# qq456cvb/CanonicalVoting

Hardware: AMD Instinct MI355X
Metric: scenes/sec (80k-pt synthetic scans) (higher is better)
Workload: dtype f32

## Files before the change

### canonicalvoting_amd/csrc/hv_vote.hip

```cpp
#include "cv_common.h"

#include <atomic>
#include <algorithm>
#include <cmath>
#include <cstddef>
#include <mutex>
#include <unordered_map>
#include <vector>

namespace {

struct F3 { float x, y, z; };
struct I3 { int x, y, z; };

std::mutex g_tab_mu;
std::unordered_map<uint64_t, float2*> g_tabs;

int get_rot_table(int num_rots, const float2** out) {
    int dev = 0;
    CV_HIP_CHECK(hipGetDevice(&dev));
    const uint64_t key = (uint64_t(uint32_t(dev)) << 32) | uint32_t(num_rots);
    std::lock_guard<std::mutex> lk(g_tab_mu);
    auto it = g_tabs.find(key);
    if (it != g_tabs.end()) { *out = it->second; return CV_OK; }
// ... 207 lines not shown
constexpr int MAX_PARTS = HV_MAX_PARTS;

template <class V, class E>
__device__ __forceinline__ int wave_excl_scan(int Y, V value, E emit) {
    const int lane = threadIdx.x & 63;
    int carry = 0;
    for (int base = 0; base < Y; base += 64) {
        const int i = base + lane;
        const int v = i < Y ? value(i) : 0;
        int incl = v;
#pragma unroll
        for (int off = 1; off < 64; off <<= 1) {
            const int t = __shfl_up(incl, off);
            if (lane >= off) incl += t;
        }
        if (i < Y) emit(i, carry + incl - v, v);
        carry += __shfl(incl, 63);
    }
    return carry;
}
__global__ __launch_bounds__(256) void hv_prep_scan(const int* __restrict__ ycount, int Y,
                                                    int* __restrict__ ystart,
                                                    int* __restrict__ cursor,
                                                    int* __restrict__ part_start, int4* __restrict__ q_info, int max_q,
                                                    int* __restrict__ chunk_start, int* __restrict__ bin_of_chunk,
                                                    int part_records, int64_t ks_ws) {
    ycount = cat_ws(ycount, ks_ws); ystart = cat_ws(ystart, ks_ws); cursor = cat_ws(cursor, ks_ws);
    part_start = cat_ws(part_start, ks_ws); q_info = cat_ws(q_info, ks_ws);
    chunk_start = cat_ws(chunk_start, ks_ws); bin_of_chunk = cat_ws(bin_of_chunk, ks_ws);
    const int wave = threadIdx.x >> 6, lane = threadIdx.x & 63;
    if (wave == 0) {
        const int total = wave_excl_scan(Y, [&](int i) { return ycount[i]; },
                                         [&](int i, int excl, int) { ystart[i] = excl; cursor[i] = excl; });
        if (lane == 0) ystart[Y] = total;
    } else if (wave == 1) {
        const int total = wave_excl_scan(Y,
            [&](int i) {
                const int n2 = (i >= 1 ? ycount[i - 1] : 0) + (i <= Y - 2 ? ycount[i] : 0);
                return min(max((n2 + part_records - 1) / part_records, 1), MAX_PARTS);
            },
            [&](int i, int excl, int v) {
                part_start[i] = excl;
                for (int p2 = 0; p2 < v; ++p2) q_info[excl + p2] = make_int4(i, p2, v, excl);
            });
        for (int q = total + lane; q < max_q; q += 64) q_info[q] = make_int4(0, 0, -1, 0);
        if (lane == 0) part_start[Y] = total;
    } else if (wave == 2) {
        const int total = wave_excl_scan(Y, [&](int i) { return (ycount[i] + LIST_CHUNK_RECORDS - 1) / LIST_CHUNK_RECORDS; },
                                         [&](int i, int excl, int v) {
                                             chunk_start[i] = excl;
                                             for (int p2 = 0; p2 < v; ++p2) bin_of_chunk[excl + p2] = i;
                                         });
        if (lane == 0) chunk_start[Y] = total;
    }
}

constexpr int REC_F = 13;

__global__ __launch_bounds__(PREP_THREADS) void hv_prep_scatter(
    const float* __restrict__ pts, const float* __restrict__ xyz, const float* __restrict__ scl,
    const float* __restrict__ obj, const int* __restrict__ fy_in, int64_t n, int Y, float res,
    F3 corner, int* __restrict__ cursor, float* __restrict__ rec, int64_t rec_stride, CatStride ks) {
    __shared__ int lh[PREP_MAX_Y];
    xyz = cat_el(xyz, 3 * ks.n); scl = cat_el(scl, 3 * ks.n); obj = cat_el(obj, ks.n);
    fy_in = cat_ws(fy_in, ks.ws); cursor = cat_ws(cursor, ks.ws); rec = cat_ws(rec, ks.ws);
    const bool use_lds = Y <= PREP_MAX_Y;
    const int64_t c = blockIdx.x * (int64_t)PREP_THREADS + threadIdx.x;
// ... 380 lines not shown
        if (ok && hi - lo > best) { best = hi - lo; best_end = (float)k * half_pi + hi; }
#pragma unroll
        for (int j = 1; j < 4; ++j) {
            const float hp = h[(k + j - 1) & 3], hn = h[(k + j) & 3];
            ok = ok && hn > 0.f && hp + hn >= half_pi;
            if (ok) {
                lo = fminf(lo, (float)j * half_pi - hn);
                hi = fmaxf(hi, (float)j * half_pi + hn);
                if (hi - lo > best) { best = hi - lo; best_end = (float)k * half_pi + hi; }
            }
        }
    }
    const float inside = fmaxf(two_pi - best, 0.f);
    const float inv_step = (float)R * 0.159154943f;
    const int len = (int)(inside * inv_step) + 6;
    if (len < a_len) {
        float first = (best_end - a0) * inv_step - 2.f;
        first -= (float)R * floorf(first / (float)R);
        a_start = min(max((int)first, 0), R - 1);
        a_len = len;
    }
}

template <int VARIANT, bool QUEUE>
__global__ __launch_bounds__(TW * 64) void hv_fwd_tiles(
    int R, float res, F3 corner, I3 dims, const float2* __restrict__ tab,
    const int* __restrict__ ystart, const int4* __restrict__ items, const float* __restrict__ rec,
    int64_t rec_stride, int tiles_x, int tiles_z, unsigned long long* __restrict__ partials,
    int* __restrict__ arrivals, float* __restrict__ g_obj, float* __restrict__ g_rot,
    float* __restrict__ g_scale, unsigned long long* __restrict__ prof,
    const int* __restrict__ list_ctl, const int* __restrict__ list_start, const int* __restrict__ list_cnt,
    const int2* __restrict__ entries, int list_mode ,
    const int4* __restrict__ q_info, CatStride ks) {
    ystart = cat_ws(ystart, ks.ws); items = cat_ws(items, ks.ws); rec = cat_ws(rec, ks.ws);
    partials = cat_ws(partials, ks.ws); arrivals = cat_ws(arrivals, ks.ws); list_ctl = cat_ws(list_ctl, ks.ws);
    list_start = cat_ws(list_start, ks.ws); list_cnt = cat_ws(list_cnt, ks.ws); entries = cat_ws(entries, ks.ws);
    q_info = cat_ws(q_info, ks.ws);
    g_obj = cat_el(g_obj, ks.cells); g_rot = cat_el(g_rot, 2 * ks.cells); g_scale = cat_el(g_scale, 3 * ks.cells);
    __shared__ TileShared sh;
    __shared__ int last_flag;
    unsigned long long pacc[8] = {0, 0, 0, 0, 0, 0, 0, 0};
    unsigned long long pt0 = VARIANT == 4 ? __builtin_amdgcn_s_memtime() : 0;
#define HV_TICK(p)                                                        \
    do {                                                                  \
        if (VARIANT == 4) {                                               \
            const unsigned long long t_ = __builtin_amdgcn_s_memtime();   \
            pacc[p] += t_ - pt0;                                          \
            pt0 = t_;                                                     \
        }                                                                 \
    } while (0)
    const int X = dims.x, Y = dims.y, Z = dims.z;
    const int ntiles = tiles_x * tiles_z;
    int y, tile, part, nparts, slot0, slot_stride;
    if (QUEUE) {
        if ((int)blockIdx.x >= list_ctl[2]) return;
        const int4 item = items[blockIdx.x];
        y = item.x; tile = item.y; part = item.z & 0xff; nparts = item.z >> 8; slot0 = item.w; slot_stride = 1;
    } else {
        tile = blockIdx.x % ntiles;
        const int4 qi = q_info[blockIdx.x / ntiles];
        if (qi.z < 0) return;
        y = qi.x; part = qi.y; nparts = qi.z;
        slot0 = qi.w * ntiles + tile; slot_stride = ntiles;
    }
    const int x0 = (tile / tiles_z) * TX, z0 = (tile % tiles_z) * TZ;
    const int lane = threadIdx.x & 63, wave = threadIdx.x >> 6;
    if (nparts == 0) {
        const int nx0 = min(TX, X - x0), nz0 = min(TZ, Z - z0);
        for (int i = threadIdx.x; i < TCELLS; i += TW * 64) {
            const int lx = i / TZ, lz = i % TZ;
            if (lx < nx0 && lz < nz0) {
                const int64_t cell = ((int64_t)(x0 + lx) * Y + y) * Z + z0 + lz;
                g_obj[cell] = 0.f;
                reinterpret_cast<float2*>(g_rot)[cell] = make_float2(0.f, 0.f);
                g_scale[cell * 3 + 0] = 0.f; g_scale[cell * 3 + 1] = 0.f; g_scale[cell * 3 + 2] = 0.f;
            }
        }
        return;
    }
    const bool use_list = QUEUE && VARIANT != 3 && list_mode == 2 && list_ctl[1] == 0;
    int lbeg[2] = {0, 0}, llen[2] = {0, 0};
    if (use_list) {
#pragma unroll
        for (int k = 0; k < 2; ++k) {
            const int s = y - 1 + k;
            if (s >= 0 && s <= Y - 2) {
                lbeg[k] = list_start[(int64_t)s * ntiles + tile];
                llen[k] = list_cnt[(int64_t)s * ntiles + tile];
            }
        }
    }

#ifdef HV_POISON
    {
        unsigned* w = reinterpret_cast<unsigned*>(&sh);
        const int lo[5] = {(int)(offsetof(TileShared, pq) / 4), (int)(offsetof(TileShared, arc_start) / 4),
                           (int)(offsetof(TileShared, arc_cum) / 4), (int)(offsetof(TileShared, vq_rec) / 4),
                           (int)(offsetof(TileShared, tab) / 4)};
        const int hi[5] = {lo[1], lo[2], lo[3], lo[4], (int)(offsetof(TileShared, next_chunk) / 4)};
        for (int k = 0; k < 5; ++k)
            if ((HV_POISON >> k) & 1)
                for (int i = lo[k] + threadIdx.x; i < hi[k]; i += TW * 64) w[i] = 0x7fc12345u + i * 2654435761u;
        __syncthreads();
    }
#endif
    int bin_beg[2], bin_end[2];
#pragma unroll
    for (int k = 0; k < 2; ++k) {
        const int s = y - 1 + k;
        const bool valid = s >= 0 && s <= Y - 2 && VARIANT != 3;
        bin_beg[k] = !valid ? 0 : (use_list ? lbeg[k] : ystart[s]);
        bin_end[k] = !valid ? 0 : (use_list ? lbeg[k] + llen[k] : ystart[s + 1]);
    }
    const float2 tab_mine = (int)threadIdx.x < R ? tab[threadIdx.x] : make_float2(0.f, 0.f);
    for (int i = threadIdx.x; i < ACC_WORDS; i += TW * 64) sh.acc[i] = 0ull;
    if ((int)threadIdx.x < R) sh.tab[threadIdx.x] = tab_mine;
    if (threadIdx.x < 2) sh.next_chunk[threadIdx.x] = 0;
    if (threadIdx.x == 2) { sh.list_len = 0; sh.more = 0; }
    __syncthreads();
    HV_TICK(0);

    const float slack = 0.05f;
    const float xlo = (float)(x0 - 1), xhi = (float)(x0 + TX), zlo = (float)(z0 - 1),
                zhi = (float)(z0 + TZ);
    int vq_len = 0;

    const int per = use_list ? LIST_CHUNK : 64;
    int sb = 0;
    int c_mask = 0, c_idx[CULL_BATCH], c_arc = 0, c_k = 0;
#pragma unroll
    for (int j = 0; j < CULL_BATCH; ++j) c_idx[j] = 0;
    auto append = [&](int mask, const int (&idx)[CULL_BATCH], int arc, int k) -> int {
        int tot = 0, before[CULL_BATCH];
#pragma unroll
        for (int j = 0; j < CULL_BATCH; ++j) {
            const uint64_t m = __ballot((mask >> j) & 1);
            before[j] = tot + lanes_below(m);
            tot += __popcll(m);
        }
        if (tot == 0) return 0;
        int p0 = 0;
        if (lane == 0) p0 = atomicAdd(&sh.list_len, tot);
        p0 = __builtin_amdgcn_readfirstlane(p0);
#pragma unroll
        for (int j = 0; j < CULL_BATCH; ++j) {
            const int pos = p0 + before[j];
            if (((mask >> j) & 1) && pos < LQ) {
                sh.arc_start[pos] = idx[j] | (int)((unsigned)k << 31);
                if (use_list) sh.arc_cum[pos] = arc;
                mask &= ~(1 << j);
            }
        }
        return mask;
    };

    for (;;) {
        bool more = false;
        if (__ballot(c_mask != 0) != 0) {
            c_mask = append(c_mask, c_idx, c_arc, c_k);
            more = __ballot(c_mask != 0) != 0;
        }
        while (!more && sb < 2) {
            if (bin_beg[sb] >= bin_end[sb]) { ++sb; continue; }
            const int len = __builtin_amdgcn_readfirstlane(
                __hip_atomic_load(&sh.list_len, __ATOMIC_RELAXED, __HIP_MEMORY_SCOPE_WORKGROUP));
            if (len > LQ - 64) { more = true; break; }
            const int take = use_list ? 64 / LIST_CHUNK : CULL_BATCH;
            int c = 0;
            if (lane == 0) c = atomicAdd(&sh.next_chunk[sb], take);
            c = __builtin_amdgcn_readfirstlane(c);
            const int end = bin_end[sb];
            if (bin_beg[sb] + (c * nparts + part) * per >= end) { ++sb; continue; }
            int idx[CULL_BATCH], mask = 0, arc = 0;
#pragma unroll
            for (int j = 0; j < CULL_BATCH; ++j) idx[j] = 0;
            if (use_list) {
                const int e = bin_beg[sb] + ((c + lane / LIST_CHUNK) * nparts + part) * LIST_CHUNK + lane % LIST_CHUNK;
                if (e < end) {
// ... 19 lines not shown
                    const float dxf = fmaxf(fabsf(ux[j] - xlo), fabsf(ux[j] - xhi));
                    const float dzf = fmaxf(fabsf(uz[j] - zlo), fabsf(uz[j] - zhi));
                    const float dmin = sqrtf(dxn * dxn + dzn * dzn), dmax = sqrtf(dxf * dxf + dzf * dzf);
                    const float tol = slack + 1e-5f * (r[j] + fabsf(ux[j]) + fabsf(uz[j]));
                    bool keep = idx[j] < end && (r[j] >= dmin - tol) && (r[j] <= dmax + tol);
                    if (VARIANT == 2) keep = keep && (ux[j] == 1234.5f);
                    mask |= (int)keep << j;
                }
            }
            c_mask = append(mask, idx, arc, sb);
            if (__ballot(c_mask != 0) != 0) {
#pragma unroll
                for (int j = 0; j < CULL_BATCH; ++j) c_idx[j] = idx[j];
                c_arc = arc; c_k = sb;
                more = true;
            }
        }
        if (more && lane == 0) sh.more = 1;
        HV_TICK(1);
        __syncthreads();
        const int n = min(sh.list_len, LQ);
        const bool again = sh.more != 0;
        HV_TICK(3);
        if (n == 0) break;

        const int p = threadIdx.x;
        int a_start = 0, a_len = 0;
        if (p < n) {
            const int w = sh.arc_start[p];
            const int idx = w & 0x7fffffff;
            if (use_list) {
                const int arc = sh.arc_cum[p];
                a_start = arc & 0xffff;
                a_len = arc >> 16;
            } else {
                const float ux = rec[9 * rec_stride + idx], uz = rec[10 * rec_stride + idx];
                const float dxn = fmaxf(0.f, fmaxf(xlo - ux, ux - xhi));
                const float dzn = fmaxf(0.f, fmaxf(zlo - uz, uz - zhi));
                a_len = R;
                if (dxn + dzn > 0.5f) {
                    const float b0 = arc_atan2(0.5f * (zlo + zhi) - uz, 0.5f * (xlo + xhi) - ux);
                    float lo = 0.f, hi = 0.f;
#pragma unroll
                    for (int k = 0; k < 4; ++k) {
                        float d = arc_atan2(((k & 2) ? zhi : zlo) - uz, ((k & 1) ? xhi : xlo) - ux) - b0;
                        d -= 6.28318531f * rintf(d * 0.159154943f);
                        lo = fminf(lo, d);
                        hi = fmaxf(hi, d);
                    }
                    const float a0 = rec[12 * rec_stride + idx];
                    const float inv_step = (float)R * 0.159154943f;
                    float first = (b0 + lo - a0) * inv_step - 2.f;
                    const int len = (int)((hi - lo) * inv_step) + 6;
                    first -= (float)R * floorf(first / (float)R);
                    a_start = min(max((int)first, 0), R - 1);
                    a_len = min(len, R);
                }
                edge_arc(ux, uz, rec[11 * rec_stride + idx], rec[12 * rec_stride + idx], R, xlo, xhi, zlo, zhi, a_start, a_len);
            }
            const float ry = rec[4 * rec_stride + idx];
            sh.pq[0][p] = rec[0 * rec_stride + idx];
            sh.pq[1][p] = rec[1 * rec_stride + idx];
            sh.pq[2][p] = rec[2 * rec_stride + idx];
            sh.pq[3][p] = rec[3 * rec_stride + idx];
            sh.pq[4][p] = (w < 0) ? (1.f - ry) : ry;
            sh.pq[5][p] = rec[5 * rec_stride + idx];
            sh.pq[6][p] = rec[6 * rec_stride + idx];
            sh.pq[7][p] = rec[7 * rec_stride + idx];
            sh.pq[8][p] = rec[8 * rec_stride + idx];
            sh.arc_start[p] = a_start;
        }
        int cum = a_len;
#pragma unroll
        for (int off = 1; off < 64; off <<= 1) {
            const int t = __shfl_up(cum, off);
            if (lane >= off) cum += t;
        }
        if (lane == 63) sh.wtot[wave] = cum;
        HV_TICK(2);
        __syncthreads();
        HV_TICK(3);
        if (threadIdx.x == 0) { sh.list_len = 0; sh.more = 0; }
        int items = 0;
#pragma unroll
        for (int w = 0; w < TW; ++w) {
            const int t = sh.wtot[w];
            if (w < wave) cum += t;
            items += t;
        }
        if (p < n) sh.arc_cum[p] = cum;
        HV_TICK(2);
        __syncthreads();
// ... 64 lines not shown
                sh.vq_rz[wave][q] = rz;
            }
            vq_len += __popcll(mv);
            wave_sync_lds();
            HV_TICK(4);
            if (vq_len >= 64) {
                vq_len -= 64;
                if (VARIANT != 1) drain64(sh, wave, vq_len + lane, true);
                HV_TICK(5);
            }
        }
        if (vq_len > 0) {
            if (VARIANT != 1) drain64(sh, wave, lane, lane < vq_len);
            else if (lane < vq_len)
                sh.acc[ACC_CH + lane] = (unsigned long long)(sh.vq_rx[wave][lane] + sh.vq_rz[wave][lane] + (float)sh.vq_rec[wave][lane]);
            vq_len = 0;
        }
        wave_sync_lds();
        HV_TICK(6);
        if (!again) break;
        __syncthreads();
        HV_TICK(3);
    }
    HV_TICK(1);
    __syncthreads();
    HV_TICK(3);

    if (nparts > 1) {
        unsigned long long* mine = partials + ((int64_t)slot0 + (int64_t)part * slot_stride) * (6 * TCELLS);
        for (int i = threadIdx.x; i < 6 * TCELLS; i += TW * 64) mine[i] = sh.acc[acc_idx(i / TCELLS, i % TCELLS)];
        asm volatile("s_waitcnt vmcnt(0)" ::: "memory");
        __syncthreads();
        if (threadIdx.x == 0) {
            __builtin_amdgcn_fence(__ATOMIC_RELEASE, "agent");
            asm volatile("s_waitcnt vmcnt(0)" ::: "memory");
            const int old = __hip_atomic_fetch_add(&arrivals[y * ntiles + tile], 1, __ATOMIC_RELAXED,
                                                   __HIP_MEMORY_SCOPE_AGENT);
            last_flag = old == nparts - 1;
            if (last_flag) __builtin_amdgcn_fence(__ATOMIC_ACQUIRE, "agent");
        }
        __syncthreads();
        if (!last_flag) return;
        const unsigned long long* base = partials + (int64_t)slot0 * (6 * TCELLS);
        for (int i = threadIdx.x; i < 6 * TCELLS; i += TW * 64) {
            unsigned long long sum = 0ull;
            for (int p2 = 0; p2 < nparts; ++p2) sum += base[(int64_t)p2 * slot_stride * (6 * TCELLS) + i];
            sh.acc[acc_idx(i / TCELLS, i % TCELLS)] = sum;
        }
        __syncthreads();
    }

    const int nx = min(TX, X - x0), nz = min(TZ, Z - z0);
    if (VARIANT == 5) {
        if (threadIdx.x == 0) g_obj[((int64_t)x0 * Y + y) * Z + z0] = (float)acc_value(sh.acc[0], 0);
        return;
    }
    for (int i = threadIdx.x; i < TCELLS; i += TW * 64) {
        const int lx = i / TZ, lz = i % TZ;
        if (lx < nx && lz < nz)
            g_obj[((int64_t)(x0 + lx) * Y + y) * Z + z0 + lz] = (float)acc_value(sh.acc[acc_idx(0, i)], 0);
    }
    for (int i = threadIdx.x; i < TCELLS * 2; i += TW * 64) {
        const int cell = i >> 1, j = i & 1;
        const int lx = cell / TZ, lz = cell % TZ;
        if (lx < nx && lz < nz) {
            const double d = (double)(float)acc_value(sh.acc[acc_idx(0, cell)], 0) + 1e-7;
            g_rot[(((int64_t)(x0 + lx) * Y + y) * Z + z0 + lz) * 2 + j] =
                (float)((double)(float)fx_value(sh.acc[acc_idx(1 + j, cell)]) / d);
        }
    }
    for (int i = threadIdx.x; i < TCELLS * 3; i += TW * 64) {
        const int cell = i / 3, j = i - cell * 3;
        const int lx = cell / TZ, lz = cell % TZ;
        if (lx < nx && lz < nz) {
            const double d = (double)(float)acc_value(sh.acc[acc_idx(0, cell)], 0) + 1e-7;
            g_scale[(((int64_t)(x0 + lx) * Y + y) * Z + z0 + lz) * 3 + j] =
                (float)((double)(float)fx_value(sh.acc[acc_idx(3 + j, cell)]) / d);
        }
    }
    HV_TICK(7);
    if (VARIANT == 4 && lane == 0) {
        for (int p2 = 0; p2 < 8; ++p2) atomicAdd(&prof[p2], pacc[p2]);
        atomicAdd(&prof[8], 1ull);
    }
#undef HV_TICK
}

__global__ __launch_bounds__(256) void hv_bwd(
    const float* __restrict__ grad, const float* __restrict__ pts, const float* __restrict__ xyz,
    const float* __restrict__ scl, const float* __restrict__ obj, int64_t n, int R, float res,
    F3 corner, I3 dims, const float2* __restrict__ tab, float* __restrict__ d_xyz,
    float* __restrict__ d_scl, float* __restrict__ d_obj) {
    const int lane = threadIdx.x & 63;
    const int64_t c = blockIdx.x * 4ll + (threadIdx.x >> 6);
    if (c >= n) return;
    const int Y = dims.y, Z = dims.z;
    const float s0 = scl[c * 3 + 0], s1 = scl[c * 3 + 1], s2 = scl[c * 3 + 2];
    const float x0 = xyz[c * 3 + 0], x1 = xyz[c * 3 + 1], x2 = xyz[c * 3 + 2];
    const float cx = x0 * s0, cy = x1 * s1, cz = x2 * s2;
    const float px = pts[c * 3 + 0], py = pts[c * 3 + 1], pz = pts[c * 3 + 2];
    const float ob = obj[c];
    float a_obj = 0, a_x0 = 0, a_x1 = 0, a_x2 = 0, a_s0 = 0, a_s1 = 0, a_s2 = 0;
    for (int i = lane; i < R; i += 64) {
        const float2 cs = tab[i];
        const float ox = (-cs.x) * cx + cs.y * cz;
        const float oy = -cy;
        const float oz = (-cs.y) * cx - cs.x * cz;
// ... 175 lines not shown
    CV_REQUIRE(res > 0.f, CV_EINVAL, "res must be positive");
    for (int k = 0; k < 3; ++k) {
        volatile float d = h_max3[k] - h_min3[k];
        volatile float q = d / res;
        dims_out[k] = (int)q + 1;
    }
    return CV_OK;
}

static bool tiles_queue_mode(int64_t n, int num_rots, int64_t Y, int64_t ntiles, int algo) {
    return use_queue(ntiles) && ntiles <= LIST_MAX_TILES && list_capacity(n, ntiles) < (1ll << 31) &&
           queue_max_items(n, num_rots, Y, ntiles) < (1ll << 31) && algo != 23;
}

size_t cv_hv_forward_workspace_bytes(int64_t n, int num_rots, const int dims[3], int algo) {
    if (!dims || n <= 0) return 0;
    if (pick_algo(algo, n, num_rots, dims) == 1) return 256;
    const size_t Y = (size_t)dims[1];
    const size_t ntiles = (size_t)((dims[0] + TX - 1) / TX) * (size_t)((dims[2] + TZ - 1) / TZ);
    const bool queue = tiles_queue_mode(n, num_rots, (int64_t)Y, (int64_t)ntiles, algo);
    const size_t max_chunks = Y + (size_t)((n + LIST_CHUNK_RECORDS - 1) / LIST_CHUNK_RECORDS);
    const size_t slots = queue ? (size_t)queue_max_slots(n, num_rots) : (size_t)tiles_q_bound(n, (int)Y) * ntiles;
    size_t b = 256 * 24 + sizeof(int) * ((size_t)n * (1 + REC_F) + Y * 8 + 16 + 64 + Y * ntiles + max_chunks +
                                         4 * (size_t)tiles_q_bound(n, (int)Y)) +
               sizeof(unsigned long long) * slots * 6 * TCELLS;
    if (queue)
        b += sizeof(int) * (3 * Y * ntiles + max_chunks * ntiles) +
             sizeof(int4) * (size_t)queue_max_items(n, num_rots, (int64_t)Y, (int64_t)ntiles) +
             sizeof(int2) * (size_t)list_capacity(n, (int64_t)ntiles);
    return b;
}

static thread_local hipEvent_t t_ev_start = nullptr, t_ev_stop = nullptr;

static std::atomic<long long> g_part_records{getenv("CV_HV_PART_RECORDS") ? std::max<long long>(PART_RECORDS, atoll(getenv("CV_HV_PART_RECORDS")))
                                                                          : (long long)PART_RECORDS};

static thread_local long long t_part_records = 0;

int cv_hv_set_part_records(int records) {
    const long long v = records <= 0 ? (long long)PART_RECORDS : std::max<long long>(PART_RECORDS, records);
    return (int)g_part_records.exchange(v, std::memory_order_relaxed);
}

int cv_hv_set_part_records_thread(int records) {
    const int before = (int)t_part_records;
    t_part_records = records <= 0 ? 0 : std::max<long long>(PART_RECORDS, records);
// ... 49 lines not shown
    const int ws_algo = algo == 23 ? 23 : 2;
    CV_REQUIRE(d_ws && ws_bytes >= cv_hv_forward_cat_workspace_bytes(n, num_rots, dims, ws_algo, K), CV_ENOMEM,
               "workspace too small for the tiles algorithm");
    const CatStride ks{K > 1 ? (int64_t)cat_ws_stride(n, num_rots, dims, ws_algo) : 0, n, cells};
    const int Y = dims[1];
    CvCarver cv(d_ws);
    int* fy = cv.take<int>(n);
    float* rec = cv.take<float>((size_t)n * REC_F);
    const int tiles_x = (dims[0] + TX - 1) / TX, tiles_z = (dims[2] + TZ - 1) / TZ;
    const int ntiles = tiles_x * tiles_z;
    const int64_t max_items = queue_max_items(n, num_rots, Y, ntiles), max_slots = queue_max_slots(n, num_rots);
    const int64_t max_q = tiles_q_bound(n, Y);
    const int64_t list_cap = list_capacity(n, ntiles);
    const bool queue = tiles_queue_mode(n, num_rots, Y, ntiles, algo);
    int* list_ctl = cv.take<int>(64);
    int* list_cnt = cv.take<int>(queue ? (size_t)Y * ntiles : 0);
    int* tile_w = cv.take<int>(queue ? (size_t)Y * ntiles : 0);
    int* ycount = cv.take<int>(Y);
    int* arrivals = cv.take<int>((size_t)Y * ntiles);
    int* ystart = cv.take<int>(Y + 1);
    int* cursor = cv.take<int>(Y);
    int* part_start = cv.take<int>(Y + 1);
    int4* q_info = cv.take<int4>((size_t)max_q);
    unsigned long long* partials = cv.take<unsigned long long>((size_t)(queue ? max_slots : max_q * ntiles) * 6 * TCELLS);
    int4* items = cv.take<int4>(queue ? (size_t)max_items : 0);
    int* list_start = cv.take<int>(queue ? (size_t)Y * ntiles : 0);
    const int64_t max_chunks = (int64_t)Y + (n + LIST_CHUNK_RECORDS - 1) / LIST_CHUNK_RECORDS;
    int* chunk_start = cv.take<int>((size_t)Y + 1);
    int* bin_of_chunk = cv.take<int>((size_t)max_chunks);
    int* chunk_off = cv.take<int>(queue ? (size_t)max_chunks * ntiles : 0);
    int2* entries = cv.take<int2>(queue ? (size_t)list_cap : 0);
    const int list_mode = queue ? 2 : 1;
    int* zero_from = queue ? list_ctl : ycount;
    const size_t zero_bytes = (size_t)(reinterpret_cast<char*>(arrivals + (size_t)Y * ntiles) - reinterpret_cast<char*>(zero_from));
    if (K == 1) CV_HIP_CHECK(hipMemsetAsync(zero_from, 0, zero_bytes, st));
    else {
        hv_zero_cat<<<dim3((unsigned)std::min<size_t>((zero_bytes / 4 + 255) / 256, 1024), K), 256, 0, st>>>(zero_from, zero_bytes / 4,
                                                                                                        ks.ws);
        CV_LAUNCH_CHECK();
    }
    const unsigned prep_wgs = (unsigned)((n + PREP_THREADS - 1) / PREP_THREADS);
    hv_prep_count<<<dim3(prep_wgs, K), PREP_THREADS, 0, st>>>(d_points, d_xyz, d_scale, n, res, corner.y, Y, fy, ycount, ks);
    CV_LAUNCH_CHECK();
    hv_prep_scan<<<dim3(1, K), 256, 0, st>>>(ycount, Y, ystart, cursor, part_start, q_info, (int)max_q, chunk_start, bin_of_chunk,
                                             (int)(t_part_records > 0 ? t_part_records : g_part_records.load(std::memory_order_relaxed)),
                                             ks.ws);
    CV_LAUNCH_CHECK();
    hv_prep_scatter<<<dim3(prep_wgs, K), PREP_THREADS, 0, st>>>(d_points, d_xyz, d_scale, d_obj, fy, n, Y, res, corner, cursor, rec,
                                                                 n, ks);
    CV_LAUNCH_CHECK();
    if (queue) {
        hv_list_pass<false><<<dim3((unsigned)max_chunks, K), 1024, 0, st>>>(ystart, chunk_start, bin_of_chunk, Y, rec, n, num_rots,
                                                                             tiles_x, tiles_z, list_ctl, list_cnt, list_start,
                                                                             chunk_off, entries, tile_w, 1, ks.ws);
        CV_LAUNCH_CHECK();
        hv_build_queue<<<dim3(1, K), 1024, 0, st>>>(tile_w, Y, ntiles, (int)max_items, (int)max_slots, list_ctl, items, ks.ws);
        CV_LAUNCH_CHECK();
        hv_list_scan<<<dim3(1, K), 1024, 0, st>>>(list_cnt, Y, ntiles, list_cap, list_ctl, list_start, ks.ws);
        CV_LAUNCH_CHECK();
        hv_list_pass<true><<<dim3((unsigned)max_chunks, K), 1024, 0, st>>>(ystart, chunk_start, bin_of_chunk, Y, rec, n, num_rots,
                                                                            tiles_x, tiles_z, list_ctl, list_cnt, list_start,
                                                                            chunk_off, entries, tile_w, 1, ks.ws);
        CV_LAUNCH_CHECK();
    }
    const int64_t wgs = queue ? max_items : max_q * ntiles;
    CV_REQUIRE(wgs < (1ll << 31), CV_EINVAL, "grid too large");
#define CV_TILES_ARGS num_rots, res, corner, d3, tab, ystart, items, rec, n, tiles_x, tiles_z, partials, arrivals, d_grid_obj, \
                      d_grid_rot, d_grid_scale, prof, list_ctl, list_start, list_cnt, entries, list_mode, q_info, ks
#define CV_TILES_LAUNCH(V)                                                                                   \
    do {                                                                                                     \
        if (t_ev_start) CV_HIP_CHECK(hipEventRecord(t_ev_start, st));                                         \
        if (queue) hv_fwd_tiles<V, true><<<dim3((unsigned)wgs, K), TW * 64, 0, st>>>(CV_TILES_ARGS);          \
        else hv_fwd_tiles<V, false><<<dim3((unsigned)wgs, K), TW * 64, 0, st>>>(CV_TILES_ARGS);               \
        if (t_ev_stop) CV_HIP_CHECK(hipEventRecord(t_ev_stop, st));                                           \
    } while (0)
    unsigned long long* prof = nullptr;
    if (algo == 24) {
        static unsigned long long* d_prof = nullptr;
        if (!d_prof) CV_HIP_CHECK(hipMalloc(&d_prof, 16 * sizeof(unsigned long long)));
        CV_HIP_CHECK(hipMemsetAsync(d_prof, 0, 16 * sizeof(unsigned long long), st));
        prof = d_prof;
        CV_TILES_LAUNCH(4);
        unsigned long long h[16];
        CV_HIP_CHECK(hipMemcpyAsync(h, d_prof, sizeof h, hipMemcpyDeviceToHost, st));
        CV_HIP_CHECK(hipStreamSynchronize(st));
        static const char* names[8] = {"init", "cull", "arcs+scan+search", "barrier-wait", "walk", "drain",
                                       "round-flush", "merge+store"};
        double tot = 0;
        for (int p2 = 0; p2 < 8; ++p2) tot += (double)h[p2];
        fprintf(stderr, "hv_fwd_tiles waves %llu ticks/wave %.0f:", h[8], tot / (double)std::max(1ull, h[8]));
        for (int p2 = 0; p2 < 8; ++p2) fprintf(stderr, " %s %.1f%%", names[p2], 100.0 * (double)h[p2] / tot);
        fprintf(stderr, "\n");
    } else
    if (algo == 25) CV_TILES_LAUNCH(5);
    else if (algo == 21) CV_TILES_LAUNCH(1);
    else if (algo == 22) CV_TILES_LAUNCH(2);
    else if (algo == 23) CV_TILES_LAUNCH(3);
    else CV_TILES_LAUNCH(0);
#undef CV_TILES_LAUNCH
#undef CV_TILES_ARGS
    CV_LAUNCH_CHECK();
    return CV_OK;
}

int cv_hv_forward_f32(const float* d_points, const float* d_xyz, const float* d_scale,
                      const float* d_obj, int64_t n, float res, int num_rots,
                      const float h_corner3[3], const int dims[3], float* d_grid_obj,
                      float* d_grid_rot, float* d_grid_scale, void* d_ws, size_t ws_bytes, int algo,
                      void* stream) {
    int rc = check_common(d_points, d_xyz, d_scale, n, res, num_rots, h_corner3, dims);
    if (rc) return rc;
    CV_REQUIRE(d_obj && d_grid_obj && d_grid_rot && d_grid_scale, CV_EINVAL, "null pointer argument");
    return hv_forward_cats(d_points, d_xyz, d_scale, d_obj, n, res, num_rots, h_corner3, dims, d_grid_obj, d_grid_rot, d_grid_scale,
                           d_ws, ws_bytes, algo, 1, static_cast<hipStream_t>(stream));
// ... 61 lines not shown
```

Baseline: 638.4.

## Skip empty tile workgroups early and fuse normalise-store into one pass

Precomputes each plane's bin record ranges (q_bins) during the prep scan, so non-queue tile workgroups whose two bins hold no records write zeros and exit before touching shared memory. Accumulator zeroing and the table load are deferred until the first non-empty list, and single-part workgroups whose cull keeps nothing also exit early with a zero store. The three separate output loops are merged into one per-cell pass that computes a double reciprocal once and multiplies by it. Record loads are hoisted ahead of the shared-memory init to overlap latency. This adds extra workspace and per-slot metadata writes, and the reciprocal-based division may differ slightly in rounding from true division.

Result: no change. 644.7 (median of 6 runs) (+1.0%).

```diff
diff --git a/canonicalvoting_amd/csrc/hv_vote.hip b/canonicalvoting_amd/csrc/hv_vote.hip
--- a/canonicalvoting_amd/csrc/hv_vote.hip
+++ b/canonicalvoting_amd/csrc/hv_vote.hip
@@ -253,11 +253,12 @@
 __global__ __launch_bounds__(256) void hv_prep_scan(const int* __restrict__ ycount, int Y,
                                                     int* __restrict__ ystart,
                                                     int* __restrict__ cursor,
-                                                    int* __restrict__ part_start, int4* __restrict__ q_info, int max_q,
+                                                    int* __restrict__ part_start, int4* __restrict__ q_info,
+                                                    int4* __restrict__ q_bins, int max_q,
                                                     int* __restrict__ chunk_start, int* __restrict__ bin_of_chunk,
                                                     int part_records, int64_t ks_ws) {
     ycount = cat_ws(ycount, ks_ws); ystart = cat_ws(ystart, ks_ws); cursor = cat_ws(cursor, ks_ws);
-    part_start = cat_ws(part_start, ks_ws); q_info = cat_ws(q_info, ks_ws);
+    part_start = cat_ws(part_start, ks_ws); q_info = cat_ws(q_info, ks_ws); q_bins = cat_ws(q_bins, ks_ws);
     chunk_start = cat_ws(chunk_start, ks_ws); bin_of_chunk = cat_ws(bin_of_chunk, ks_ws);
     const int wave = threadIdx.x >> 6, lane = threadIdx.x & 63;
     if (wave == 0) {
@@ -265,15 +266,30 @@
                                          [&](int i, int excl, int) { ystart[i] = excl; cursor[i] = excl; });
         if (lane == 0) ystart[Y] = total;
     } else if (wave == 1) {
-        const int total = wave_excl_scan(Y,
-            [&](int i) {
-                const int n2 = (i >= 1 ? ycount[i - 1] : 0) + (i <= Y - 2 ? ycount[i] : 0);
-                return min(max((n2 + part_records - 1) / part_records, 1), MAX_PARTS);
-            },
-            [&](int i, int excl, int v) {
+        int total = 0, rec_carry = 0;
+        for (int base = 0; base < Y; base += 64) {
+            const int i = base + lane;
+            const int c_below = (i >= 1 && i < Y) ? ycount[i - 1] : 0, c_all = i < Y ? ycount[i] : 0;
+            const int c_here = i <= Y - 2 ? c_all : 0;
+            const int v = i < Y ? min(max((c_below + c_here + part_records - 1) / part_records, 1), MAX_PARTS) : 0;
+            int incl = v, rec_incl = c_all;
+#pragma unroll
+            for (int off = 1; off < 64; off <<= 1) {
+                const int t = __shfl_up(incl, off), tr = __shfl_up(rec_incl, off);
+                if (lane >= off) { incl += t; rec_incl += tr; }
+            }
+            if (i < Y) {
+                const int excl = total + incl - v, b1 = rec_carry + rec_incl - c_all;
                 part_start[i] = excl;
-                for (int p2 = 0; p2 < v; ++p2) q_info[excl + p2] = make_int4(i, p2, v, excl);
-            });
+                const int4 bins = make_int4(b1 - c_below, b1, b1 + c_here, 0);
+                for (int p2 = 0; p2 < v; ++p2) {
+                    q_info[excl + p2] = make_int4(i, p2, v, excl);
+                    q_bins[excl + p2] = bins;
+                }
+            }
+            total += __shfl(incl, 63);
+            rec_carry += __shfl(rec_incl, 63);
+        }
         for (int q = total + lane; q < max_q; q += 64) q_info[q] = make_int4(0, 0, -1, 0);
         if (lane == 0) part_start[Y] = total;
     } else if (wave == 2) {
@@ -700,6 +716,60 @@
     }
 }
 
+
+__device__ __forceinline__ void zero_acc(TileShared& sh) {
+    for (int i = threadIdx.x; i < ACC_WORDS; i += TW * 64) sh.acc[i] = 0ull;
+}
+
+__device__ __forceinline__ void store_zero_tile(int x0, int z0, int y, I3 dims, float* __restrict__ g_obj,
+                                                float* __restrict__ g_rot, float* __restrict__ g_scale) {
+    const int nx = min(TX, dims.x - x0), nz = min(TZ, dims.z - z0);
+    for (int i = threadIdx.x; i < TCELLS; i += TW * 64) {
+        const int lx = i / TZ, lz = i % TZ;
+        if (lx < nx && lz < nz) {
+            const int64_t cell = ((int64_t)(x0 + lx) * dims.y + y) * dims.z + z0 + lz;
+            g_obj[cell] = 0.f;
+            reinterpret_cast<float2*>(g_rot)[cell] = make_float2(0.f, 0.f);
+            g_scale[cell * 3 + 0] = 0.f; g_scale[cell * 3 + 1] = 0.f; g_scale[cell * 3 + 2] = 0.f;
+        }
+    }
+}
+
+__device__ __forceinline__ double div_reciprocal(double d) {
+    double r = __builtin_amdgcn_rcp(d);
+    double e = __builtin_fma(-d, r, 1.0);
+    r = __builtin_fma(r, e, r);
+    e = __builtin_fma(-d, r, 1.0);
+    return __builtin_fma(r, e, r);
+}
+__device__ __forceinline__ double div_by(double n, double d, double r) {
+    const double q = n * r;
+    return __builtin_fma(__builtin_fma(-d, q, n), r, q);
+}
+
+__device__ __forceinline__ void normalise_store_tile(const TileShared& sh, int x0, int z0, int y, I3 dims,
+                                                     float* __restrict__ g_obj, float* __restrict__ g_rot,
+                                                     float* __restrict__ g_scale) {
+    const int nx = min(TX, dims.x - x0), nz = min(TZ, dims.z - z0);
+    for (int i = threadIdx.x; i < TCELLS; i += TW * 64) {
+        const int lx = i / TZ, lz = i % TZ;
+        if (lx < nx && lz < nz) {
+            const unsigned long long* a = sh.acc + acc_idx(0, i);
+            const float wf = (float)fx_value(a[0]);
+            const double d = (double)wf + 1e-7;
+            const double r = div_reciprocal(d);
+            float q[5];
+#pragma unroll
+            for (int j = 0; j < 5; ++j) q[j] = (float)div_by((double)(float)fx_value(a[(1 + j) * ACC_CH]), d, r);
+            const int64_t cell = ((int64_t)(x0 + lx) * dims.y + y) * dims.z + z0 + lz;
+            g_obj[cell] = wf;
+            reinterpret_cast<float2*>(g_rot)[cell] = make_float2(q[0], q[1]);
+            g_scale[cell * 3 + 0] = q[2]; g_scale[cell * 3 + 1] = q[3]; g_scale[cell * 3 + 2] = q[4];
+        }
+    }
+}
+
+constexpr int PROF_PHASES = 10;
 template <int VARIANT, bool QUEUE>
 __global__ __launch_bounds__(TW * 64) void hv_fwd_tiles(
     int R, float res, F3 corner, I3 dims, const float2* __restrict__ tab,
@@ -709,15 +779,16 @@
     float* __restrict__ g_scale, unsigned long long* __restrict__ prof,
     const int* __restrict__ list_ctl, const int* __restrict__ list_start, const int* __restrict__ list_cnt,
     const int2* __restrict__ entries, int list_mode ,
-    const int4* __restrict__ q_info, CatStride ks) {
+    const int4* __restrict__ q_info, const int4* __restrict__ q_bins, CatStride ks) {
     ystart = cat_ws(ystart, ks.ws); items = cat_ws(items, ks.ws); rec = cat_ws(rec, ks.ws);
     partials = cat_ws(partials, ks.ws); arrivals = cat_ws(arrivals, ks.ws); list_ctl = cat_ws(list_ctl, ks.ws);
     list_start = cat_ws(list_start, ks.ws); list_cnt = cat_ws(list_cnt, ks.ws); entries = cat_ws(entries, ks.ws);
-    q_info = cat_ws(q_info, ks.ws);
+    q_info = cat_ws(q_info, ks.ws); q_bins = cat_ws(q_bins, ks.ws);
     g_obj = cat_el(g_obj, ks.cells); g_rot = cat_el(g_rot, 2 * ks.cells); g_scale = cat_el(g_scale, 3 * ks.cells);
     __shared__ TileShared sh;
     __shared__ int last_flag;
-    unsigned long long pacc[8] = {0, 0, 0, 0, 0, 0, 0, 0};
+    constexpr bool EXIT = VARIANT != 2 && VARIANT != 3;
+    unsigned long long pacc[PROF_PHASES] = {};
     unsigned long long pt0 = VARIANT == 4 ? __builtin_amdgcn_s_memtime() : 0;
 #define HV_TICK(p)                                                        \
     do {                                                                  \
@@ -730,30 +801,32 @@
     const int X = dims.x, Y = dims.y, Z = dims.z;
     const int ntiles = tiles_x * tiles_z;
     int y, tile, part, nparts, slot0, slot_stride;
+    int4 qb = make_int4(0, 0, 0, 0);
     if (QUEUE) {
         if ((int)blockIdx.x >= list_ctl[2]) return;
         const int4 item = items[blockIdx.x];
         y = item.x; tile = item.y; part = item.z & 0xff; nparts = item.z >> 8; slot0 = item.w; slot_stride = 1;
     } else {
         tile = blockIdx.x % ntiles;
-        const int4 qi = q_info[blockIdx.x / ntiles];
+        const int slot = blockIdx.x / ntiles;
+        const int4 qi = q_info[slot];
+        qb = q_bins[slot];
         if (qi.z < 0) return;
         y = qi.x; part = qi.y; nparts = qi.z;
         slot0 = qi.w * ntiles + tile; slot_stride = ntiles;
     }
     const int x0 = (tile / tiles_z) * TX, z0 = (tile % tiles_z) * TZ;
     const int lane = threadIdx.x & 63, wave = threadIdx.x >> 6;
-    if (nparts == 0) {
-        const int nx0 = min(TX, X - x0), nz0 = min(TZ, Z - z0);
-        for (int i = threadIdx.x; i < TCELLS; i += TW * 64) {
-            const int lx = i / TZ, lz = i % TZ;
-            if (lx < nx0 && lz < nz0) {
-                const int64_t cell = ((int64_t)(x0 + lx) * Y + y) * Z + z0 + lz;
-                g_obj[cell] = 0.f;
-                reinterpret_cast<float2*>(g_rot)[cell] = make_float2(0.f, 0.f);
-                g_scale[cell * 3 + 0] = 0.f; g_scale[cell * 3 + 1] = 0.f; g_scale[cell * 3 + 2] = 0.f;
-            }
-        }
+    auto prof_flush = [&]() {
+        if (VARIANT == 4 && lane == 0) {
+            for (int p2 = 0; p2 < PROF_PHASES; ++p2) atomicAdd(&prof[p2], pacc[p2]);
+            atomicAdd(&prof[PROF_PHASES], 1ull);
+        }
+    };
+    if (nparts == 0 || (!QUEUE && EXIT && qb.x == qb.z)) {
+        store_zero_tile(x0, z0, y, dims, g_obj, g_rot, g_scale);
+        HV_TICK(9);
+        prof_flush();
         return;
     }
     const bool use_list = QUEUE && VARIANT != 3 && list_mode == 2 && list_ctl[1] == 0;
@@ -787,12 +860,14 @@
     for (int k = 0; k < 2; ++k) {
         const int s = y - 1 + k;
         const bool valid = s >= 0 && s <= Y - 2 && VARIANT != 3;
-        bin_beg[k] = !valid ? 0 : (use_list ? lbeg[k] : ystart[s]);
-        bin_end[k] = !valid ? 0 : (use_list ? lbeg[k] + llen[k] : ystart[s + 1]);
-    }
-    const float2 tab_mine = (int)threadIdx.x < R ? tab[threadIdx.x] : make_float2(0.f, 0.f);
-    for (int i = threadIdx.x; i < ACC_WORDS; i += TW * 64) sh.acc[i] = 0ull;
-    if ((int)threadIdx.x < R) sh.tab[threadIdx.x] = tab_mine;
+        if (QUEUE) {
+            bin_beg[k] = !valid ? 0 : (use_list ? lbeg[k] : ystart[s]);
+            bin_end[k] = !valid ? 0 : (use_list ? lbeg[k] + llen[k] : ystart[s + 1]);
+        } else {
+            bin_beg[k] = VARIANT == 3 ? 0 : (k == 0 ? qb.x : qb.y);
+            bin_end[k] = VARIANT == 3 ? 0 : (k == 0 ? qb.y : qb.z);
+        }
+    }
     if (threadIdx.x < 2) sh.next_chunk[threadIdx.x] = 0;
     if (threadIdx.x == 2) { sh.list_len = 0; sh.more = 0; }
     __syncthreads();
@@ -832,6 +907,8 @@
         return mask;
     };
 
+    bool first = true;
+    bool empty = false;
     for (;;) {
         bool more = false;
         if (__ballot(c_mask != 0) != 0) {
@@ -897,19 +974,48 @@
         const int n = min(sh.list_len, LQ);
         const bool again = sh.more != 0;
         HV_TICK(3);
-        if (n == 0) break;
+        if (n == 0) {
+            if (first) {
+                empty = true;
+            }
+            break;
+        }
 
         const int p = threadIdx.x;
-        int a_start = 0, a_len = 0;
+        int a_start = 0, a_len = 0, w = 0;
+        float f[9] = {0.f, 0.f, 0.f, 0.f, 0.f, 0.f, 0.f, 0.f, 0.f}, ux = 0.f, uz = 0.f, rr = 0.f, a0 = 0.f;
         if (p < n) {
-            const int w = sh.arc_start[p];
+            w = sh.arc_start[p];
             const int idx = w & 0x7fffffff;
+#pragma unroll
+            for (int k = 0; k < 9; ++k) f[k] = rec[k * rec_stride + idx];
+            if (!use_list) {
+                ux = rec[9 * rec_stride + idx]; uz = rec[10 * rec_stride + idx];
+                rr = rec[11 * rec_stride + idx]; a0 = rec[12 * rec_stride + idx];
+            }
+        }
+        if (first) {
+            const float2 tab_mine = (int)threadIdx.x < R ? tab[threadIdx.x] : make_float2(0.f, 0.f);
+            zero_acc(sh);
+            if ((int)threadIdx.x < R) sh.tab[threadIdx.x] = tab_mine;
+            first = false;
+            HV_TICK(8);
+        }
+        if (p < n) {
+            sh.pq[0][p] = f[0];
+            sh.pq[1][p] = f[1];
+            sh.pq[2][p] = f[2];
+            sh.pq[3][p] = f[3];
+            sh.pq[4][p] = (w < 0) ? (1.f - f[4]) : f[4];
+            sh.pq[5][p] = f[5];
+            sh.pq[6][p] = f[6];
+            sh.pq[7][p] = f[7];
+            sh.pq[8][p] = f[8];
             if (use_list) {
                 const int arc = sh.arc_cum[p];
                 a_start = arc & 0xffff;
                 a_len = arc >> 16;
             } else {
-                const float ux = rec[9 * rec_stride + idx], uz = rec[10 * rec_stride + idx];
                 const float dxn = fmaxf(0.f, fmaxf(xlo - ux, ux - xhi));
                 const float dzn = fmaxf(0.f, fmaxf(zlo - uz, uz - zhi));
                 a_len = R;
@@ -923,26 +1029,15 @@
                         lo = fminf(lo, d);
                         hi = fmaxf(hi, d);
                     }
-                    const float a0 = rec[12 * rec_stride + idx];
                     const float inv_step = (float)R * 0.159154943f;
-                    float first = (b0 + lo - a0) * inv_step - 2.f;
+                    float first_rot = (b0 + lo - a0) * inv_step - 2.f;
                     const int len = (int)((hi - lo) * inv_step) + 6;
-                    first -= (float)R * floorf(first / (float)R);
-                    a_start = min(max((int)first, 0), R - 1);
+                    first_rot -= (float)R * floorf(first_rot / (float)R);
+                    a_start = min(max((int)first_rot, 0), R - 1);
                     a_len = min(len, R);
                 }
-                edge_arc(ux, uz, rec[11 * rec_stride + idx], rec[12 * rec_stride + idx], R, xlo, xhi, zlo, zhi, a_start, a_len);
-            }
-            const float ry = rec[4 * rec_stride + idx];
-            sh.pq[0][p] = rec[0 * rec_stride + idx];
-            sh.pq[1][p] = rec[1 * rec_stride + idx];
-            sh.pq[2][p] = rec[2 * rec_stride + idx];
-            sh.pq[3][p] = rec[3 * rec_stride + idx];
-            sh.pq[4][p] = (w < 0) ? (1.f - ry) : ry;
-            sh.pq[5][p] = rec[5 * rec_stride + idx];
-            sh.pq[6][p] = rec[6 * rec_stride + idx];
-            sh.pq[7][p] = rec[7 * rec_stride + idx];
-            sh.pq[8][p] = rec[8 * rec_stride + idx];
+                edge_arc(ux, uz, rr, a0, R, xlo, xhi, zlo, zhi, a_start, a_len);
+            }
             sh.arc_start[p] = a_start;
         }
         int cum = a_len;
@@ -1053,6 +1148,16 @@
         __syncthreads();
         HV_TICK(3);
     }
+    if (empty) {
+        if (EXIT && nparts == 1) {
+            store_zero_tile(x0, z0, y, dims, g_obj, g_rot, g_scale);
+            HV_TICK(9);
+            prof_flush();
+            return;
+        }
+        zero_acc(sh);
+        HV_TICK(8);
+    }
     HV_TICK(1);
     __syncthreads();
     HV_TICK(3);
@@ -1081,39 +1186,13 @@
         __syncthreads();
     }
 
-    const int nx = min(TX, X - x0), nz = min(TZ, Z - z0);
     if (VARIANT == 5) {
         if (threadIdx.x == 0) g_obj[((int64_t)x0 * Y + y) * Z + z0] = (float)acc_value(sh.acc[0], 0);
         return;
     }
-    for (int i = threadIdx.x; i < TCELLS; i += TW * 64) {
-        const int lx = i / TZ, lz = i % TZ;
-        if (lx < nx && lz < nz)
-            g_obj[((int64_t)(x0 + lx) * Y + y) * Z + z0 + lz] = (float)acc_value(sh.acc[acc_idx(0, i)], 0);
-    }
-    for (int i = threadIdx.x; i < TCELLS * 2; i += TW * 64) {
-        const int cell = i >> 1, j = i & 1;
-        const int lx = cell / TZ, lz = cell % TZ;
-        if (lx < nx && lz < nz) {
-            const double d = (double)(float)acc_value(sh.acc[acc_idx(0, cell)], 0) + 1e-7;
-            g_rot[(((int64_t)(x0 + lx) * Y + y) * Z + z0 + lz) * 2 + j] =
-                (float)((double)(float)fx_value(sh.acc[acc_idx(1 + j, cell)]) / d);
-        }
-    }
-    for (int i = threadIdx.x; i < TCELLS * 3; i += TW * 64) {
-        const int cell = i / 3, j = i - cell * 3;
-        const int lx = cell / TZ, lz = cell % TZ;
-        if (lx < nx && lz < nz) {
-            const double d = (double)(float)acc_value(sh.acc[acc_idx(0, cell)], 0) + 1e-7;
-            g_scale[(((int64_t)(x0 + lx) * Y + y) * Z + z0 + lz) * 3 + j] =
-                (float)((double)(float)fx_value(sh.acc[acc_idx(3 + j, cell)]) / d);
-        }
-    }
+    normalise_store_tile(sh, x0, z0, y, dims, g_obj, g_rot, g_scale);
     HV_TICK(7);
-    if (VARIANT == 4 && lane == 0) {
-        for (int p2 = 0; p2 < 8; ++p2) atomicAdd(&prof[p2], pacc[p2]);
-        atomicAdd(&prof[8], 1ull);
-    }
+    prof_flush();
 #undef HV_TICK
 }
 
@@ -1335,7 +1414,7 @@
     const size_t max_chunks = Y + (size_t)((n + LIST_CHUNK_RECORDS - 1) / LIST_CHUNK_RECORDS);
     const size_t slots = queue ? (size_t)queue_max_slots(n, num_rots) : (size_t)tiles_q_bound(n, (int)Y) * ntiles;
     size_t b = 256 * 24 + sizeof(int) * ((size_t)n * (1 + REC_F) + Y * 8 + 16 + 64 + Y * ntiles + max_chunks +
-                                         4 * (size_t)tiles_q_bound(n, (int)Y)) +
+                                         8 * (size_t)tiles_q_bound(n, (int)Y)) +
                sizeof(unsigned long long) * slots * 6 * TCELLS;
     if (queue)
         b += sizeof(int) * (3 * Y * ntiles + max_chunks * ntiles) +
@@ -1431,6 +1510,7 @@
     int* cursor = cv.take<int>(Y);
     int* part_start = cv.take<int>(Y + 1);
     int4* q_info = cv.take<int4>((size_t)max_q);
+    int4* q_bins = cv.take<int4>((size_t)max_q);
     unsigned long long* partials = cv.take<unsigned long long>((size_t)(queue ? max_slots : max_q * ntiles) * 6 * TCELLS);
     int4* items = cv.take<int4>(queue ? (size_t)max_items : 0);
     int* list_start = cv.take<int>(queue ? (size_t)Y * ntiles : 0);
@@ -1451,7 +1531,8 @@
     const unsigned prep_wgs = (unsigned)((n + PREP_THREADS - 1) / PREP_THREADS);
     hv_prep_count<<<dim3(prep_wgs, K), PREP_THREADS, 0, st>>>(d_points, d_xyz, d_scale, n, res, corner.y, Y, fy, ycount, ks);
     CV_LAUNCH_CHECK();
-    hv_prep_scan<<<dim3(1, K), 256, 0, st>>>(ycount, Y, ystart, cursor, part_start, q_info, (int)max_q, chunk_start, bin_of_chunk,
+    hv_prep_scan<<<dim3(1, K), 256, 0, st>>>(ycount, Y, ystart, cursor, part_start, q_info, q_bins, (int)max_q, chunk_start,
+                                             bin_of_chunk,
                                              (int)(t_part_records > 0 ? t_part_records : g_part_records.load(std::memory_order_relaxed)),
                                              ks.ws);
     CV_LAUNCH_CHECK();
@@ -1475,7 +1556,7 @@
     const int64_t wgs = queue ? max_items : max_q * ntiles;
     CV_REQUIRE(wgs < (1ll << 31), CV_EINVAL, "grid too large");
 #define CV_TILES_ARGS num_rots, res, corner, d3, tab, ystart, items, rec, n, tiles_x, tiles_z, partials, arrivals, d_grid_obj, \
-                      d_grid_rot, d_grid_scale, prof, list_ctl, list_start, list_cnt, entries, list_mode, q_info, ks
+                      d_grid_rot, d_grid_scale, prof, list_ctl, list_start, list_cnt, entries, list_mode, q_info, q_bins, ks
 #define CV_TILES_LAUNCH(V)                                                                                   \
     do {                                                                                                     \
         if (t_ev_start) CV_HIP_CHECK(hipEventRecord(t_ev_start, st));                                         \
@@ -1493,12 +1574,13 @@
         unsigned long long h[16];
         CV_HIP_CHECK(hipMemcpyAsync(h, d_prof, sizeof h, hipMemcpyDeviceToHost, st));
         CV_HIP_CHECK(hipStreamSynchronize(st));
-        static const char* names[8] = {"init", "cull", "arcs+scan+search", "barrier-wait", "walk", "drain",
-                                       "round-flush", "merge+store"};
+        static_assert(PROF_PHASES + 1 <= 16, "d_prof holds the phases and the wave count");
+        static const char* names[PROF_PHASES] = {"init", "cull", "arcs+scan+search", "barrier-wait", "walk", "drain",
+                                                 "round-flush", "merge+store", "zero-acc", "empty-exit"};
         double tot = 0;
-        for (int p2 = 0; p2 < 8; ++p2) tot += (double)h[p2];
-        fprintf(stderr, "hv_fwd_tiles waves %llu ticks/wave %.0f:", h[8], tot / (double)std::max(1ull, h[8]));
-        for (int p2 = 0; p2 < 8; ++p2) fprintf(stderr, " %s %.1f%%", names[p2], 100.0 * (double)h[p2] / tot);
+        for (int p2 = 0; p2 < PROF_PHASES; ++p2) tot += (double)h[p2];
+        fprintf(stderr, "hv_fwd_tiles waves %llu ticks/wave %.0f:", h[PROF_PHASES], tot / (double)std::max(1ull, h[PROF_PHASES]));
+        for (int p2 = 0; p2 < PROF_PHASES; ++p2) fprintf(stderr, " %s %.1f%%", names[p2], 100.0 * (double)h[p2] / tot);
         fprintf(stderr, "\n");
     } else
     if (algo == 25) CV_TILES_LAUNCH(5);
diff --git a/profiles/vote_fixed_cost_pricing.py b/profiles/vote_fixed_cost_pricing.py
--- /dev/null
+++ b/profiles/vote_fixed_cost_pricing.py
@@ -0,0 +1,147 @@
+import os
+import sys
+
+import numpy as np
+
+sys.path.insert(0, os.path.dirname(os.path.dirname(os.path.abspath(__file__))))
+from canonicalvoting_amd.synth import make_scene, synth_predictions
+
+f32 = np.float32
+R, RES, TX, TZ, MAX_PARTS = 120, f32(0.03), 16, 32, 8
+PART_SIZES = (4096, 12288)
+
+
+def scene_counts(seed, n_points=80000):
+    sc = make_scene(seed, n_points=n_points)
+    xyz, scale, prob, _ = synth_predictions(sc)
+    pts = sc.points.astype(f32)
+    corner = pts.min(0)
+    X, Y, Z = (int(v) for v in (np.trunc((pts.max(0) - corner) / RES) + 1))
+    c = (xyz * scale).astype(f32)
+    gy = ((pts[:, 1] - c[:, 1] - corner[1]) / RES).astype(f32)
+    fy = np.where((gy >= 0) & (gy < Y - 1), gy.astype(np.int64), -1)
+    ux, uz = ((pts[:, 0] - corner[0]) / RES).astype(f32), ((pts[:, 2] - corner[2]) / RES).astype(f32)
+    rad = (np.sqrt(c[:, 0] * c[:, 0] + c[:, 2] * c[:, 2]) / RES).astype(f32)
+    tx, tz = -(-X // TX), -(-Z // TZ)
+
+    theta = (np.arange(R, dtype=f32) * f32(2 * 3.141592654 / R)).astype(f32)
+    cs, sn = np.cos(theta.astype(np.float64)).astype(f32), np.sin(theta.astype(np.float64)).astype(f32)
+    ox = ((-cs[None]) * c[:, 0:1] + sn[None] * c[:, 2:3]).astype(f32)
+    oz = ((-sn[None]) * c[:, 0:1] - cs[None] * c[:, 2:3]).astype(f32)
+    gx = (((pts[:, 0:1] + ox) - corner[0]) / RES).astype(f32)
+    gz = (((pts[:, 2:3] + oz) - corner[2]) / RES).astype(f32)
+    gyb = np.broadcast_to(gy[:, None], gx.shape)
+    inb = (gx >= 0) & (gz >= 0) & (gyb >= 0) & (gx < X - 1) & (gz < Z - 1) & (gyb < Y - 1)
+    ix, iy, iz = gx[inb].astype(np.int64), gyb[inb].astype(np.int64), gz[inb].astype(np.int64)
+    touched = np.zeros((X + 1, Y + 1, Z + 1), bool)
+    for dx in (0, 1):
+        for dy in (0, 1):
+            for dz in (0, 1):
+                touched[ix + dx, iy + dy, iz + dz] = True
+    touched = touched[:X, :Y, :Z]
+    pad = np.zeros((tx * TX, Y, tz * TZ), bool)
+    pad[:X, :, :Z] = touched
+    wg_cells = pad.reshape(tx, TX, Y, tz, TZ).transpose(0, 3, 2, 1, 4)
+    wg_any = wg_cells.any((3, 4))
+    groups = wg_cells.reshape(tx, tz, Y, TX // 2, 2 * TZ).any(4)
+
+    nrec = np.zeros(Y, np.int64)
+    kept = {}
+    bbox = np.zeros((Y, tx, tz), bool)
+    for s in range(Y - 1):
+        idx = np.flatnonzero(fy == s)
+        nrec[s] = len(idx)
+        if not len(idx):
+            continue
+        bux, buz, br = ux[idx], uz[idx], rad[idx]
+        bx0, bx1 = (bux - br).min() - 1, (bux + br).max() + 1
+        bz0, bz1 = (buz - br).min() - 1, (buz + br).max() + 1
+        for a in range(tx):
+            for b in range(tz):
+                x0, z0 = a * TX, b * TZ
+                xlo, xhi, zlo, zhi = f32(x0 - 1), f32(x0 + TX), f32(z0 - 1), f32(z0 + TZ)
+                dxn = np.maximum(f32(0), np.maximum(xlo - bux, bux - xhi))
+                dzn = np.maximum(f32(0), np.maximum(zlo - buz, buz - zhi))
+                dxf = np.maximum(np.abs(bux - xlo), np.abs(bux - xhi))
+                dzf = np.maximum(np.abs(buz - zlo), np.abs(buz - zhi))
+                dmin, dmax = np.sqrt(dxn * dxn + dzn * dzn), np.sqrt(dxf * dxf + dzf * dzf)
+                tol = f32(0.05) + f32(1e-5) * (br + np.abs(bux) + np.abs(buz))
+                kept[(s, a, b)] = np.flatnonzero((br >= dmin - tol) & (br <= dmax + tol))
+                bbox[s, a, b] = not (xhi < bx0 or xlo > bx1 or zhi < bz0 or zlo > bz1)
+
+    out = dict(grid="%d x %d x %d" % (X, Y, Z), tiles="%d x %d" % (tx, tz))
+    wgs = empty = empty_culls = culls = small = bb = 0
+    live = np.zeros(Y, bool)
+    parts = {pr: dict(wgs=0, empty=0, planes_split=0, max_parts=0) for pr in PART_SIZES}
+    for y in range(Y):
+        bins = [s for s in (y - 1, y) if 0 <= s <= Y - 2]
+        n2 = int(sum(nrec[s] for s in bins))
+        if n2 == 0:
+            continue
+        live[y] = True
+        for a in range(tx):
+            for b in range(tz):
+                wgs += 1
+                n = sum(len(kept[(s, a, b)]) for s in bins if nrec[s])
+                ch = sum(-(-int(nrec[s]) // 64) for s in bins)
+                culls += ch
+                if n == 0:
+                    empty += 1
+                    empty_culls += ch
+                    bb += not any(bbox[s, a, b] for s in bins)
+                elif n <= 64:
+                    small += 1
+                for pr in PART_SIZES:
+                    P = min(max(-(-n2 // pr), 1), MAX_PARTS)
+                    has = np.zeros(P, bool)
+                    for s in bins:
+                        if nrec[s]:
+                            has[(kept[(s, a, b)] // 64) % P] = True
+                    parts[pr]["wgs"] += P
+                    parts[pr]["empty"] += int((~has).sum())
+        for pr in PART_SIZES:
+            P = min(max(-(-n2 // pr), 1), MAX_PARTS)
+            parts[pr]["planes_split"] += P > 1
+            parts[pr]["max_parts"] = max(parts[pr]["max_parts"], P)
+    la, lg, lc = wg_any[:, :, live], groups[:, :, live], wg_cells[:, :, live]
+    out.update(planes_with_records="%d of %d" % (int(live.sum()), Y), wgs=wgs, empty=empty, empty_culls=empty_culls, culls=culls,
+               small=small, bbox=bb, touched=float(touched.mean()), untouched_wgs=int((~la).sum()),
+               untouched_groups_in_touched_wgs=float((~lg[la]).mean()), untouched_groups=float((~lg).mean()),
+               touched_in_live=float(lc.mean()), parts=parts, ntiles=tx * tz)
+    return out
+
+
+if __name__ == "__main__":
+    seeds = [int(a) for a in sys.argv[1:]] or [0, 1]
+    cols = [scene_counts(s) for s in seeds]
+    pct = lambda a, b: "%d (%.1f %%)" % (a, 100.0 * a / b)
+    rows = [
+        ("grid cells", lambda c: c["grid"]),
+        ("tiles", lambda c: c["tiles"]),
+        ("planes whose two bins hold a record", lambda c: c["planes_with_records"]),
+        ("(tile, plane) workgroups of those planes", lambda c: "%d" % c["wgs"]),
+        ("workgroups whose cull keeps no record", lambda c: pct(c["empty"], c["wgs"])),
+        ("workgroups without a touched cell", lambda c: pct(c["untouched_wgs"], c["wgs"])),
+        ("share of all chunk culls the no-record workgroups run", lambda c: "%.1f %%" % (100.0 * c["empty_culls"] / c["culls"])),
+        ("workgroups with 1..64 survivors", lambda c: pct(c["small"], c["wgs"])),
+        ("grid cells touched by any vote", lambda c: "%.1f %%" % (100 * c["touched"])),
+        ("cells of the (padded) tiles of those planes that are touched", lambda c: "%.1f %%" % (100 * c["touched_in_live"])),
+        ("untouched 64-cell store groups, all those workgroups", lambda c: "%.1f %%" % (100 * c["untouched_groups"])),
+        ("untouched 64-cell store groups inside touched workgroups", lambda c: "%.1f %%" % (100 * c["untouched_groups_in_touched_wgs"])),
+        ("no-record workgroups a per-bin ring bounding box catches", lambda c: "%d" % c["bbox"]),
+    ]
+    print("hv_fwd_tiles, streaming launch, %d rotations, %d x %d-cell tiles, 80 000-point bench scenes" % (R, TX, TZ))
+    print("%-64s %s" % ("quantity", "".join("%22s" % ("scene %d" % s) for s in seeds)))
+    for name, fn in rows:
+        print("%-64s %s" % (name, "".join("%22s" % fn(c) for c in cols)))
+    for pr in PART_SIZES:
+        print("\n== part split at %d records per part (parts of a plane = ceil(records of its two bins / %d), 1..%d)" % (pr, pr, MAX_PARTS))
+        prow = [
+            ("planes split into more than one part", lambda c: "%d" % c["parts"][pr]["planes_split"]),
+            ("most parts of a plane", lambda c: "%d" % c["parts"][pr]["max_parts"]),
+            ("(tile, plane, part) workgroups", lambda c: "%d" % c["parts"][pr]["wgs"]),
+            ("workgroups per tile (= (plane, part) slots)", lambda c: "%d" % (c["parts"][pr]["wgs"] // c["ntiles"])),
+            ("parts whose cull keeps no record", lambda c: pct(c["parts"][pr]["empty"], c["parts"][pr]["wgs"])),
+        ]
+        for name, fn in prow:
+            print("%-64s %s" % (name, "".join("%22s" % fn(c) for c in cols)))
diff --git a/profiles/vote_kernel_alone.py b/profiles/vote_kernel_alone.py
--- /dev/null
+++ b/profiles/vote_kernel_alone.py
@@ -0,0 +1,60 @@
+import argparse
+import os
+import statistics
+import sys
+
+import numpy as np
+import torch
+
+sys.path.insert(0, os.path.dirname(os.path.dirname(os.path.abspath(__file__))))
+from canonicalvoting_amd import _lib, hv_cuda
+from canonicalvoting_amd.hough import HoughVoting
+from canonicalvoting_amd.synth import make_scene, synth_predictions
+
+ap = argparse.ArgumentParser()
+ap.add_argument("--seeds", default="0,1")
+ap.add_argument("--parts", default="4096,12288")
+ap.add_argument("--launches", type=int, default=25)
+ap.add_argument("--no-ticks", action="store_true")
+a = ap.parse_args()
+dev = torch.device("cuda:0")
+L = _lib.lib()
+t = lambda x: torch.from_numpy(np.ascontiguousarray(x)).to(dev)
+hv = HoughVoting(0.03, 120)
+ev = [torch.cuda.Event(enable_timing=True) for _ in range(2)]
+for e in ev:
+    e.record()
+torch.cuda.synchronize()
+for seed in (int(s) for s in a.seeds.split(",")):
+    sc = make_scene(seed, n_points=80000)
+    xyz, scale, prob, _ = synth_predictions(sc)
+    args = (t(sc.points), t(xyz), t(scale), t(prob))
+    for records in (int(p) for p in a.parts.split(",")):
+        before = L.cv_hv_set_part_records_thread(records)
+        try:
+            with torch.no_grad():
+                for _ in range(5):
+                    hv(*args)
+                torch.cuda.synchronize()
+                us = []
+                L.cv_hv_set_kernel_events(ev[0].cuda_event, ev[1].cuda_event)
+                try:
+                    for _ in range(a.launches):
+                        hv(*args)
+                        torch.cuda.synchronize()
+                        us.append(1e3 * ev[0].elapsed_time(ev[1]))
+                finally:
+                    L.cv_hv_set_kernel_events(None, None)
+            print("seed %d part_records %d hv_fwd_tiles us: median %.1f min %.1f max %.1f" % (
+                seed, records, statistics.median(us), min(us), max(us)), flush=True)
+            if not a.no_ticks:
+                hv_cuda.set_algorithm(24)
+                try:
+                    with torch.no_grad():
+                        for _ in range(2):
+                            hv(*args)
+                    torch.cuda.synchronize()
+                finally:
+                    hv_cuda.set_algorithm(0)
+        finally:
+            L.cv_hv_set_part_records_thread(before)
```
